# justinkay/aldi

Measured on AMD Instinct MI355X. Metric: images/sec (student+teacher ALDI step), R50-FPN 1333x800, higher is better.
Workload: dtype bf16

## Files before the change

### aldi_amd/csrc/elementwise.hip

```cpp
#include "common.h"
#include <stdlib.h>

namespace {

template <typename T>
__global__ void dgrad_weights_kernel(const float* __restrict__ w, const float* __restrict__ scale, T* __restrict__ wt,
                                     int Cout, int KH, int KW, int Cin) {
    long total = (long)Cout * KH * KW * Cin;
    for (long i = blockIdx.x * (long)blockDim.x + threadIdx.x; i < total; i += (long)gridDim.x * blockDim.x) {
        int co = (int)(i % Cout);
        long r = i / Cout;
        int kw = (int)(r % KW); r /= KW;
        int kh = (int)(r % KH);
        int ci = (int)(r / KH);
        float v = w[(((long)co * KH + (KH - 1 - kh)) * KW + (KW - 1 - kw)) * Cin + ci];
        if (scale) v *= scale[co];
        Elem<T>::st(wt + i, v);
    }
}

template <typename T>
__global__ __launch_bounds__(256) void dgrad_weights_batch_kernel(const aldi_dgw_item* __restrict__ items, int n_items) {
    __shared__ float tl[32][33];
    const int tile = blockIdx.x;
    int it = 0, hi = n_items - 1;
    while (it < hi) {
        const int mid = (it + hi + 1) >> 1;
        if (items[mid].tile_begin <= tile) it = mid;
        else hi = mid - 1;
    }
    const aldi_dgw_item d = items[it];
    const int Cout = d.Cout, KH = d.KH, KW = d.KW, Cin = d.Cin, T_ = KH * KW;
    const int nci = (Cin + 31) >> 5, nco = (Cout + 31) >> 5;
    int t = tile - d.tile_begin;
    const int cit = t % nci; t /= nci;
    const int cot = t % nco;
    const int tap = t / nco;
    const int kh = tap / KW, kw = tap - kh * KW;
    const int stap = (KH - 1 - kh) * KW + (KW - 1 - kw);
    const int tx = threadIdx.x & 31, ty = threadIdx.x >> 5;
#pragma unroll
    for (int k = 0; k < 4; ++k) {
        const int co = cot * 32 + ty + k * 8, ci = cit * 32 + tx;
        float v = 0.f;
        if (co < Cout && ci < Cin) {
            v = d.w_master[((long)co * T_ + stap) * Cin + ci];
            if (d.scale) v *= d.scale[co];
        }
        tl[ty + k * 8][tx] = v;
    }
    __syncthreads();
    T* __restrict__ wt = static_cast<T*>(d.wt);
#pragma unroll
    for (int k = 0; k < 4; ++k) {
        const int ci = cit * 32 + ty + k * 8, co = cot * 32 + tx;
        if (co < Cout && ci < Cin) Elem<T>::st(wt + ((long)ci * T_ + tap) * Cout + co, tl[tx][ty + k * 8]);
    }
}

struct StemDev {
    const uint8_t* img;
    const float* w;
    const float* scale; const float* shift;
    void* y;
    int N, Hs, Ws, Hc, Wc;
    int h[ALDI_MAX_IMAGES], wd[ALDI_MAX_IMAGES];
    float mean[3], inv_std[3];
};

template <typename T>
__global__ __launch_bounds__(256) void stem_kernel(StemDev p) {
    constexpr int TI = 16 * 2 + 5;
    __shared__ float ws[147 * 64];
    __shared__ float tile[3 * TI * TI];
    const int n = blockIdx.z;
    const int oy0 = blockIdx.y * 16, ox0 = blockIdx.x * 16;
    for (int i = threadIdx.x; i < 147 * 64; i += 256) {
        int co = i & 63, tap = i >> 6;
        ws[i] = p.w[co * 147 + tap];
    }
    const int iy0 = oy0 * 2 - 3, ix0 = ox0 * 2 - 3;
    const int h = p.h[n], w = p.wd[n];
    for (int i = threadIdx.x; i < 3 * TI * TI; i += 256) {
        int c = i / (TI * TI), r = i - c * TI * TI;
        int yy = r / TI, xx = r - yy * TI;
        int iy = iy0 + yy, ix = ix0 + xx;
        float v = 0.f;
        if (iy >= 0 && iy < h && ix >= 0 && ix < w)
            v = ((float)p.img[(((long)n * 3 + c) * p.Hs + iy) * p.Ws + ix] - p.mean[c]) * p.inv_std[c];
        tile[i] = v;
    }
    __syncthreads();
    const int ty = threadIdx.x >> 4, tx = threadIdx.x & 15;
    const int oy = oy0 + ty, ox = ox0 + tx;
    float acc[64];
#pragma unroll
    for (int i = 0; i < 64; ++i) acc[i] = 0.f;
    for (int kh = 0; kh < 7; ++kh)
        for (int kw = 0; kw < 7; ++kw)
#pragma unroll
            for (int c = 0; c < 3; ++c) {
                float xv = tile[(c * TI + ty * 2 + kh) * TI + tx * 2 + kw];
                const float4* wr = reinterpret_cast<const float4*>(&ws[((kh * 7 + kw) * 3 + c) * 64]);
#pragma unroll
                for (int q = 0; q < 16; ++q) {
                    float4 wv = wr[q];
                    acc[q * 4 + 0] = fmaf(xv, wv.x, acc[q * 4 + 0]);
                    acc[q * 4 + 1] = fmaf(xv, wv.y, acc[q * 4 + 1]);
                    acc[q * 4 + 2] = fmaf(xv, wv.z, acc[q * 4 + 2]);
                    acc[q * 4 + 3] = fmaf(xv, wv.w, acc[q * 4 + 3]);
                }
            }
    if (oy < p.Hc && ox < p.Wc) {
        T* out = static_cast<T*>(p.y) + (((long)n * p.Hc + oy) * p.Wc + ox) * 64;
#pragma unroll
        for (int q = 0; q < 16; ++q) {
            float v[4];
#pragma unroll
            for (int r = 0; r < 4; ++r) {
                float t = acc[q * 4 + r] * p.scale[q * 4 + r] + p.shift[q * 4 + r];
                v[r] = t > 0.f ? t : 0.f;
            }
            store4(out + q * 4, v);
        }
    }
}

__global__ __launch_bounds__(256) void stem_mfma_kernel(StemDev p) {
    constexpr int TH = 37, TW = 40, WK = 200;
    __shared__ __attribute__((aligned(16))) bf16_t wl[64 * WK];
    __shared__ __attribute__((aligned(16))) bf16_t tile[3 * TH * TW];
    const int n = blockIdx.z;
    const int oy0 = blockIdx.y * 16, ox0 = blockIdx.x * 16;
    for (int i = threadIdx.x; i < 64 * 192; i += 256) {
        const int co = i / 192, k = i - co * 192;
        const int idx = k >> 3, kw = k & 7;
        float v = 0.f;
        if (idx < 21 && kw < 7) {
            const int c = idx / 7, kh = idx - c * 7;
// ... 631 lines not shown
    }
    ALDI_CHECK_LAUNCH();
    return ALDI_OK;
}

extern "C" int aldi_upsample2_bwd(const void* g, void* out, int N, int Hc, int Wc, int C, int accumulate, int dtype, aldi_stream_t stream) {
    long total = (long)N * Hc * Wc * (C / 4);
    hipStream_t st = static_cast<hipStream_t>(stream);
    if (dtype == ALDI_BF16) hipLaunchKernelGGL(upsample2_bwd_kernel<bf16_t>, dim3(nblocks(total)), dim3(256), 0, st, (const bf16_t*)g, (bf16_t*)out, N, Hc, Wc, C, accumulate);
    else hipLaunchKernelGGL(upsample2_bwd_kernel<float>, dim3(nblocks(total)), dim3(256), 0, st, (const float*)g, (float*)out, N, Hc, Wc, C, accumulate);
    ALDI_CHECK_LAUNCH();
    return ALDI_OK;
}

extern "C" int aldi_upsample2_bwd_chain(const void* g2, void* o3, void* o4, void* o5, int N, int H5, int W5, int C, int dtype, aldi_stream_t stream) {
    if (!g2 || !o3 || !o4 || !o5 || N < 1 || H5 < 1 || W5 < 1 || (C & 3)) return aldi_set_error_msg(ALDI_ERR_ARG, "upsample2_bwd_chain: bad args");
    const long total = (long)N * H5 * W5 * (C / 4);
    hipStream_t st = static_cast<hipStream_t>(stream);
    if (dtype == ALDI_BF16) hipLaunchKernelGGL(upsample2_bwd_chain_kernel<bf16_t>, dim3(cdiv(total, 256)), dim3(256), 0, st, (const bf16_t*)g2, (bf16_t*)o3, (bf16_t*)o4, (bf16_t*)o5, N, H5, W5, C);
    else hipLaunchKernelGGL(upsample2_bwd_chain_kernel<float>, dim3(cdiv(total, 256)), dim3(256), 0, st, (const float*)g2, (float*)o3, (float*)o4, (float*)o5, N, H5, W5, C);
    ALDI_CHECK_LAUNCH();
    return ALDI_OK;
}

extern "C" int aldi_add_f32(const void* a, const float* b, const void* relu_src, void* out, long n, int dtype, aldi_stream_t stream) {
    if (n % 4) return aldi_set_error_msg(ALDI_ERR_ARG, "add_f32: n must be a multiple of 4");
    hipStream_t st = static_cast<hipStream_t>(stream);
    if (dtype == ALDI_BF16) hipLaunchKernelGGL(add_f32_kernel<bf16_t>, dim3(nblocks(n / 4)), dim3(256), 0, st, (const bf16_t*)a, b, (const bf16_t*)relu_src, (bf16_t*)out, n / 4);
    else hipLaunchKernelGGL(add_f32_kernel<float>, dim3(nblocks(n / 4)), dim3(256), 0, st, (const float*)a, b, (const float*)relu_src, (float*)out, n / 4);
    ALDI_CHECK_LAUNCH();
    return ALDI_OK;
}

extern "C" int aldi_cast_from_f32(const float* src, void* dst, long n, int dtype, aldi_stream_t stream) {
    hipStream_t st = static_cast<hipStream_t>(stream);
    if (dtype == ALDI_BF16) hipLaunchKernelGGL(cast_from_f32_kernel<bf16_t>, dim3(nblocks(n)), dim3(256), 0, st, src, (bf16_t*)dst, n);
    else hipLaunchKernelGGL(cast_from_f32_kernel<float>, dim3(nblocks(n)), dim3(256), 0, st, src, (float*)dst, n);
    ALDI_CHECK_LAUNCH();
    return ALDI_OK;
}

extern "C" int aldi_sgd_step(float* p, const float* g, float* buf, void* p_compute, long n, float lr, float momentum, float weight_decay,
                             float grad_scale, int first_step, int dtype, aldi_stream_t stream) {
    if (!p || !g || !buf) return aldi_set_error_msg(ALDI_ERR_ARG, "sgd_step: null pointer");
    hipStream_t st = static_cast<hipStream_t>(stream);
    if (dtype == ALDI_BF16) hipLaunchKernelGGL(sgd_kernel<bf16_t>, dim3(nblocks(n)), dim3(256), 0, st, p, g, buf, (bf16_t*)p_compute, n, lr, momentum, weight_decay, grad_scale, first_step);
    else hipLaunchKernelGGL(sgd_kernel<float>, dim3(nblocks(n)), dim3(256), 0, st, p, g, buf, (float*)nullptr, n, lr, momentum, weight_decay, grad_scale, first_step);
    ALDI_CHECK_LAUNCH();
    return ALDI_OK;
}

extern "C" int aldi_sgd_step_dev(float* p, const float* g, float* buf, void* p_compute, long n, const float* hyper, int dtype, aldi_stream_t stream) {
    if (!p || !g || !buf || !hyper || n <= 0) return aldi_set_error_msg(ALDI_ERR_ARG, "sgd_step_dev: bad args");
    hipStream_t st = static_cast<hipStream_t>(stream);
    if (dtype == ALDI_BF16) hipLaunchKernelGGL(sgd_dev_kernel<bf16_t>, dim3(nblocks(n)), dim3(256), 0, st, p, g, buf, (bf16_t*)p_compute, n, hyper);
    else hipLaunchKernelGGL(sgd_dev_kernel<float>, dim3(nblocks(n)), dim3(256), 0, st, p, g, buf, (float*)nullptr, n, hyper);
    ALDI_CHECK_LAUNCH();
    return ALDI_OK;
}

extern "C" int aldi_ema_update(float* teacher, const float* student, void* teacher_compute, long n, long n_compute, double alpha, int copy_only, int dtype,
                               aldi_stream_t stream) {
    if (!teacher || !student) return aldi_set_error_msg(ALDI_ERR_ARG, "ema_update: null pointer");
    hipStream_t st = static_cast<hipStream_t>(stream);
    const float oma = (float)(1.0 - alpha);
    const float alpha_f = (float)alpha;
    const long nc = teacher_compute ? (n_compute < n ? n_compute : n) : 0;
    const int cap = aldi_tuning().ema_blocks > 0 ? aldi_tuning().ema_blocks : 16384;
    if (dtype == ALDI_BF16) hipLaunchKernelGGL(ema_kernel<bf16_t>, dim3(nblocks(n / 4 + 1, 256, cap)), dim3(256), 0, st, teacher, student, (bf16_t*)teacher_compute, n, nc, oma, alpha_f, copy_only);
    else hipLaunchKernelGGL(ema_kernel<float>, dim3(nblocks(n / 4 + 1, 256, cap)), dim3(256), 0, st, teacher, student, (float*)nullptr, n, 0L, oma, alpha_f, copy_only);
    ALDI_CHECK_LAUNCH();
    return ALDI_OK;
}

extern "C" int aldi_bn_fold(const float* w, const float* b, const float* mean, const float* var, float* scale, float* shift, int C, aldi_stream_t stream) {
    hipLaunchKernelGGL(bn_fold_kernel, dim3(cdiv(C, 256)), dim3(256), 0, static_cast<hipStream_t>(stream), w, b, mean, var, scale, shift, C, 1e-5f);
    ALDI_CHECK_LAUNCH();
    return ALDI_OK;
}

extern "C" int aldi_dgrad_weights_batch(const aldi_dgw_item* items, int n_items, int total_tiles, int dtype, aldi_stream_t stream) {
    if (!items || n_items <= 0 || total_tiles <= 0) return aldi_set_error_msg(ALDI_ERR_ARG, "dgrad_weights_batch: bad args");
    hipStream_t st = static_cast<hipStream_t>(stream);
    if (dtype == ALDI_BF16) hipLaunchKernelGGL(dgrad_weights_batch_kernel<bf16_t>, dim3(total_tiles), dim3(256), 0, st, items, n_items);
    else if (dtype == ALDI_F32) hipLaunchKernelGGL(dgrad_weights_batch_kernel<float>, dim3(total_tiles), dim3(256), 0, st, items, n_items);
    else return aldi_set_error_msg(ALDI_ERR_ARG, "dgrad_weights_batch: bad dtype");
    ALDI_CHECK_LAUNCH();
    return ALDI_OK;
}

extern "C" int aldi_dgrad_weights(const float* w_master, const float* scale, void* wt, int Cout, int KH, int KW, int Cin,
                                  int dtype, aldi_stream_t stream) {
    if (!w_master || !wt) return aldi_set_error_msg(ALDI_ERR_ARG, "dgrad_weights: null pointer");
    long total = (long)Cout * KH * KW * Cin;
    int blocks = (int)((total + 255) / 256);
    if (blocks > 8192) blocks = 8192;
    hipStream_t st = static_cast<hipStream_t>(stream);
    if (dtype == ALDI_BF16) hipLaunchKernelGGL(dgrad_weights_kernel<bf16_t>, dim3(blocks), dim3(256), 0, st, w_master, scale, (bf16_t*)wt, Cout, KH, KW, Cin);
    else hipLaunchKernelGGL(dgrad_weights_kernel<float>, dim3(blocks), dim3(256), 0, st, w_master, scale, (float*)wt, Cout, KH, KW, Cin);
    ALDI_CHECK_LAUNCH();
    return ALDI_OK;
}
```

### aldi_amd/csrc/host.h

```cpp
#pragma once
#include "../../include/aldi_hip.h"

int aldi_set_error_msg(int code, const char* msg);

typedef uint16_t bf16_t;

#define ALDI_KNOBS(X) \
    X(igemm_xcd, 1) X(igemm_tile, 0) X(igemm_dbg, 0) X(igemm_bigtile_min, 1024) X(igemm_bigtile, 64) X(igemm_bigtile_k, 768) X(igemm_lintile_min, 768) \
    X(igemm_halo, 1) X(igemm_force, 0) X(igemm_k64_min, 1024) X(igemm_group, 1) X(igemm_narrow_k, 512) X(igemm_splitk_tile, 2) X(igemm_halo_f32, 0) \
    X(igemm_f32_tile64_max, 4096) X(igemm_direct, 15) X(igemm_lean, 1) X(igemm_halo64_mid, 0) X(igemm_ws, 1) X(igemm_ws_wgs, 512) X(igemm_ws_min, 40000) \
    X(wgrad_lean, 1) X(wgrad_big_min, 28) X(wgrad_big_slots, 256) X(wgrad_slots, 384) X(wgrad_xcd, 1) \
    X(igemm_halo_ilv, 1) X(igemm_halo_small, 0) X(igemm_halo96, 0) \
    X(wgrad_dma, 0) X(wgrad_dbg, 0) X(wgrad_group_slots, 0) X(wgrad_group_epi, 24) X(wgrad_db, 0) X(wgrad_ordered, 1) X(wgrad_big_group, 1) X(wgrad_big_epi, 12) \
    X(wgrad_big_group_min, 64) X(wgrad_lds_pad_kb, 0) X(wgrad_f32_tile128, 1) X(wgrad_dma64, 3) X(wgrad_ilv, 0) \
    X(msda_gather, 7) X(msda_gather_list, 1500) X(msda_bin, 1) X(msda_bin_list, 512) X(roialign_sep, 1) X(roialign_bwd_rows, 2) \
    X(colsum_blocks, 256) X(colsum_minrows, 16) X(colsum_nt, 1024) X(colsum_block_kb, 384) \
    X(stem_mfma, 1) X(stem_pool_wgs, 0) X(sab_blocks, 512) X(ln_bwd_blocks, 512) X(ln_bwd_blocks_narrow, 1024) X(rpn_topk_fused, 1) X(ema_blocks, 2048) X(nms_mask_tri, 1) X(match_wave, 1)

struct AldiTuning {
#define ALDI_KNOB_FIELD(name, dflt) int name;
    ALDI_KNOBS(ALDI_KNOB_FIELD)
#undef ALDI_KNOB_FIELD
};
AldiTuning& aldi_tuning();
void aldi_note_dispatch(const char* kernel);

static inline int cdiv(long a, long b) { return (int)((a + b - 1) / b); }
```

### aldi_amd/csrc/wgrad.hip

```cpp
#include "common.h"
#include "wgrad_select.h"
#include <hip/amd_detail/amd_hip_unsafe_atomics.h>
#include <stdio.h>
#include <stdlib.h>

namespace {

__device__ __forceinline__ int swz8(int row, int c) { return c ^ ((row >> 1) & 7); }

__device__ __forceinline__ void transpose8x8_b16(const uint4 in[8], uint4 out[8]) {
    const uint32_t* r = reinterpret_cast<const uint32_t*>(in);
    uint32_t* o = reinterpret_cast<uint32_t*>(out);
#pragma unroll
    for (int d = 0; d < 4; ++d)
#pragma unroll
        for (int j = 0; j < 4; ++j) {
            uint32_t a = r[(2 * j) * 4 + d], b = r[(2 * j + 1) * 4 + d];
            o[(2 * d) * 4 + j] = (a & 0xffffu) | (b << 16);
            o[(2 * d + 1) * 4 + j] = (a >> 16) | (b & 0xffff0000u);
        }
}

__global__ __launch_bounds__(256) void wgrad_bf16_kernel(WgDev p) {
    constexpr int BP = 64;
// ... 311 lines not shown
#pragma unroll
                for (int j = 0; j < 4; ++j) {
                    const uint32_t a = rr[(2 * j) * 4 + d], b = rr[(2 * j + 1) * 4 + d];
                    oo[(2 * d) * 4 + j] = __builtin_amdgcn_perm(b, a, 0x05040100u);
                    oo[(2 * d + 1) * 4 + j] = __builtin_amdgcn_perm(b, a, 0x07060302u);
                }
        }
        if constexpr (!DB) __syncthreads();
        uint4* img = DB ? lds + ((p0 - pbeg) / BP & 1) * ((TCO + TKK) * 8) : lds;
#pragma unroll
        for (int c = 0; c < 8; ++c) img[iw + c * 8 + (wu ^ (c >> 1))] = out[c];
        if (p0 + BP < pend) load_slab();
        __syncthreads();
#pragma unroll
        for (int ks = 0; ks < 2; ++ks) {
            uint4 af[TM], bfr[TN];
            const int ia = ia0 ^ (ks * 4), ib = ib0 ^ (ks * 4);
#pragma unroll
            for (int i = 0; i < TM; ++i) af[i] = img[ia + i * 128];
#pragma unroll
            for (int j = 0; j < TN; ++j) bfr[j] = img[ib + j * 128];
#pragma unroll
            for (int i = 0; i < TM; ++i)
#pragma unroll
                for (int j = 0; j < TN; ++j)
                    acc[i][j] = __builtin_amdgcn_mfma_f32_16x16x32_bf16(*reinterpret_cast<bf16x8_t*>(&af[i]),
                                                                         *reinterpret_cast<bf16x8_t*>(&bfr[j]), acc[i][j], 0, 0, 0);
            if (do_bias) {
#pragma unroll
                for (int i = 0; i < TM; ++i)
                    accb[i] = __builtin_amdgcn_mfma_f32_16x16x32_bf16(*reinterpret_cast<bf16x8_t*>(&af[i]), *reinterpret_cast<const bf16x8_t*>(&ones4), accb[i], 0, 0, 0);
            }
        }
    }
    wgrad_finish_tile<TCO, TKK, WM, WN>(p, acc, accb, do_bias, bx, by, bz, wave, lane);
}

__global__ __launch_bounds__(256) __attribute__((amdgpu_waves_per_eu(3))) void wgrad_bf16_lean_kernel(WgDev p) {
    __shared__ uint4 lds[2 * 128 * 8];
    wgrad_bf16_lean_body<128, 128, 2, 2>(p, lds);
}
__device__ __forceinline__ void wgrad_group_pick(const WgGroup& G, int& i, int& tx, int& ty, int& bz) {
    const int W = G.wg_begin[G.n];
    int g = (int)blockIdx.x;
    if (G.p[0].xcd) {
        const int q = W >> 3, r = W & 7, xcd = g & 7, idx = g >> 3;
        g = (xcd < r ? xcd * (q + 1) : r * (q + 1) + (xcd - r) * q) + idx;
    }
    i = 0;
    for (int k = 1; k < G.n; ++k)
        if (g >= G.wg_begin[k]) i = k;
    i = __builtin_amdgcn_readfirstlane(i);
    const int local = g - G.wg_begin[i];
    const int tiles = G.gx[i] * G.gy[i];
    const int t = local % tiles;
    bz = local / tiles;
    tx = t % G.gx[i]; ty = t / G.gx[i];
}
__global__ __launch_bounds__(256) __attribute__((amdgpu_waves_per_eu(3))) void wgrad_bf16_lean_group_kernel(WgGroup G) {
    __shared__ uint4 lds[2 * 128 * 8];
    int i, tx, ty, bz;
    wgrad_group_pick(G, i, tx, ty, bz);
    wgrad_bf16_lean_tile<128, 128, 2, 2>(G.p[i], lds, tx, ty, bz);
}

__global__ __launch_bounds__(256) void wgrad_bf16_lean_group_db_kernel(WgGroup G) {
    __shared__ uint4 lds[2 * 2 * 128 * 8];
    int i, tx, ty, bz;
    wgrad_group_pick(G, i, tx, ty, bz);
    wgrad_bf16_lean_tile<128, 128, 2, 2, true>(G.p[i], lds, tx, ty, bz);
}

__global__ __launch_bounds__(512) void wgrad_bf16_big_kernel(WgDev p) {
    __shared__ uint4 lds[2 * 256 * 8];
    wgrad_bf16_lean_body<256, 256, 2, 4>(p, lds);
}
__global__ __launch_bounds__(512) void wgrad_bf16_big_group_kernel(WgGroup G) {
    __shared__ uint4 lds[2 * 256 * 8];
    int i, tx, ty, bz;
    wgrad_group_pick(G, i, tx, ty, bz);
    wgrad_bf16_lean_tile<256, 256, 2, 4>(G.p[i], lds, tx, ty, bz);
}

template <int TCO, int TKK, int WM, int WN>
__device__ __forceinline__ void wgrad_finalize_part(const WgFinItem& it, int local) {
    constexpr int TM = TCO / WM / 16, TN = TKK / WN / 16, NW = WM * WN, NF = TM * TN, HALVES = NW / 4;
    const int S = it.S;
    const int nblk = it.gx * it.gy * NF * HALVES;
    if (local >= nblk) {
        if (!it.db || local > nblk) return;
        for (int co = threadIdx.x; co < it.Cout; co += 256) {
            const float* b = it.wsb + (long)(co / TCO) * S * TCO + co % TCO;
            float sum = 0.f;
            for (int k = 0; k < S; ++k) sum += b[(long)k * TCO];
            it.db[co] += sum;
        }
        return;
    }
    const int h = local % HALVES, f = (local / HALVES) % NF, t = local / (HALVES * NF);
    const int wave = h * 4 + (int)(threadIdx.x >> 6), lane = threadIdx.x & 63;
    const float4* src = reinterpret_cast<const float4*>(it.ws) + (((long)t * S) * NW + wave) * (long)(NF * 64) + f * 64 + lane;
    float4 sum = make_float4(0.f, 0.f, 0.f, 0.f);
    int k = 0;
    for (; k + 4 <= S; k += 4) {
        const float4 v0 = src[(long)(k + 0) * NW * NF * 64], v1 = src[(long)(k + 1) * NW * NF * 64];
        const float4 v2 = src[(long)(k + 2) * NW * NF * 64], v3 = src[(long)(k + 3) * NW * NF * 64];
        sum.x += v0.x; sum.y += v0.y; sum.z += v0.z; sum.w += v0.w;
        sum.x += v1.x; sum.y += v1.y; sum.z += v1.z; sum.w += v1.w;
        sum.x += v2.x; sum.y += v2.y; sum.z += v2.z; sum.w += v2.w;
        sum.x += v3.x; sum.y += v3.y; sum.z += v3.z; sum.w += v3.w;
    }
    for (; k < S; ++k) {
        const float4 v = src[(long)k * NW * NF * 64];
        sum.x += v.x; sum.y += v.y; sum.z += v.z; sum.w += v.w;
    }
    const int bx = t % it.gx, by = t / it.gx, wm = wave / WN, wn = wave % WN, i = f / TN, j = f % TN, fr = lane & 15, fq = lane >> 4;
    const int kk = by * TKK + wn * (TKK / WN) + j * 16 + fr;
    if (kk >= it.K) return;
    const float v[4] = {sum.x, sum.y, sum.z, sum.w};
#pragma unroll
    for (int r = 0; r < 4; ++r) {
        const int co = bx * TCO + wm * (TCO / WM) + i * 16 + fq * 4 + r;
        if (co < it.Cout) it.dw[(long)co * it.K + kk] += v[r] * (it.scale ? it.scale[co] : 1.f);
    }
}
__global__ __launch_bounds__(256) void wgrad_finalize_kernel(WgFin F) {
    const int bid = (int)blockIdx.x;
    int i = 0;
    for (int k = 1; k < F.n; ++k)
        if (bid >= F.wg_begin[k]) i = k;
    i = __builtin_amdgcn_readfirstlane(i);
    const int local = bid - F.wg_begin[i];
    if (F.it[i].big) wgrad_finalize_part<256, 256, 2, 4>(F.it[i], local);
    else wgrad_finalize_part<128, 128, 2, 2>(F.it[i], local);
}

typedef unsigned int u32x4 __attribute__((ext_vector_type(4)));
__device__ __forceinline__ void glds16w(__amdgpu_buffer_rsrc_t rsrc, void* dst, unsigned voff) {
    __builtin_amdgcn_raw_ptr_buffer_load_lds(rsrc, (__attribute__((address_space(3))) void*)dst, 16, voff, 0, 0, 0);
}
typedef unsigned int u32x2_t __attribute__((ext_vector_type(2)));
template <int OFF>
__device__ __forceinline__ u32x2_t tr_read(unsigned addr) {
    u32x2_t v;
    asm volatile("ds_read_b64_tr_b16 %0, %1 offset:%2" : "=v"(v) : "v"(addr), "n"(OFF));
    return v;
}
template <int N, int I = 0>
__device__ __forceinline__ void tr_read_frags(u32x2_t* lo, u32x2_t* hi, unsigned addr) {
    if constexpr (I < N) {
        lo[I] = tr_read<I * 1024>(addr);
        hi[I] = tr_read<I * 1024 + 512>(addr);
        tr_read_frags<N, I + 1>(lo, hi, addr);
    }
}

template <int TCO, int TKK, int WM, int WN>
__global__ __launch_bounds__(WM* WN * 64) void wgrad_bf16_dma_kernel(WgDev p) {
    constexpr int NW = WM * WN, NT = NW * 64;
    constexpr int BP = 32;
    constexpr int GB = TCO / 16, XB = TKK / 16;
    constexpr int NBLK = GB + XB;
    static_assert(NBLK % NW == 0, "every wave issues the same number of DMA instructions per slab");
    constexpr int PER_WAVE = NBLK / NW;
    constexpr int TM = TCO / WM / 16, TN = TKK / WN / 16;
    constexpr int NBUF = 3;
    constexpr int STAGE = NBLK * 1024;
    __shared__ __attribute__((aligned(1024))) unsigned char lds[NBUF * STAGE];

    const int tid = threadIdx.x, lane = tid & 63, wave = __builtin_amdgcn_readfirstlane(tid >> 6);
    int bx = blockIdx.x, by = blockIdx.y, bz = blockIdx.z;
    {
        const int gx = gridDim.x, gy = gridDim.y, total = gx * gy * gridDim.z;
        int bid = bx + gx * (by + gy * bz);
        if (p.xcd) {
            const int q = total >> 3, r = total & 7, xcd = bid & 7, idx = bid >> 3;
            bid = (xcd < r ? xcd * (q + 1) : r * (q + 1) + (xcd - r) * q) + idx;
        }
        bx = bid % gx; bid /= gx;
        by = bid % gy; bz = bid / gy;
    }
    const int co0 = bx * TCO, kk0 = by * TKK;
    const int pbeg = bz * p.pix_per_split;
    const int pend = min(p.M, pbeg + p.pix_per_split);
    if (pbeg >= pend) return;

    constexpr unsigned OOB = 0x80000000u;
    const __amdgpu_buffer_rsrc_t rg = make_rsrc_uniform(p.g, min((unsigned)pend * (unsigned)p.Cout * 2u, p.g_bytes));
    const __amdgpu_buffer_rsrc_t rx = make_rsrc_uniform(p.x, p.x_bytes);

    const int lp = lane >> 1, lh = lane & 1;
    unsigned voff[PER_WAVE];
    int tapbit[PER_WAVE];
#pragma unroll
    for (int k = 0; k < PER_WAVE; ++k) {
        const int b = wave * PER_WAVE + k;
        tapbit[k] = -1;
        if (b < GB) {
            const int ch = co0 + b * 16 + lh * 8;
            voff[k] = ch < p.Cout ? ((unsigned)(pbeg + lp) * (unsigned)p.Cout + (unsigned)ch) * 2u : OOB;
        } else {
            const int ch = kk0 + (b - GB) * 16 + lh * 8;
            if (ch >= p.K) { voff[k] = OOB; continue; }
            const int tap = ch / p.Cin, ci = ch - tap * p.Cin;
            const int kh = tap / p.KW, kw = tap - kh * p.KW;
            voff[k] = ((unsigned)(pbeg + lp + (kh - p.pad) * p.W + (kw - p.pad)) * (unsigned)p.Cin + (unsigned)ci) * 2u;
            if (!p.ident) tapbit[k] = tap;
        }
    }
    int ph = 0, pw = 0;
    if (!p.ident) {
        const int r = (pbeg + lp) % (p.H * p.W);
        ph = r / p.W; pw = r - ph * p.W;
    }
    const unsigned x_row = (unsigned)p.Cin * 2u, g_row = (unsigned)p.Cout * 2u;
    int ld_pix = pbeg;

// ... 508 lines not shown
    float acc[EP];
#pragma unroll
    for (int k = 0; k < EP; ++k) acc[k] = 0.f;
    auto add = [&](const uint4& v) {
        if constexpr (EP == 8) {
            const uint32_t* w = reinterpret_cast<const uint32_t*>(&v);
#pragma unroll
            for (int k = 0; k < 4; ++k) { acc[2 * k] += __uint_as_float(w[k] << 16); acc[2 * k + 1] += __uint_as_float(w[k] & 0xffff0000u); }
        } else {
            const float* w = reinterpret_cast<const float*>(&v);
#pragma unroll
            for (int k = 0; k < 4; ++k) acc[k] += w[k];
        }
    };
    if (lane_r < rl) {
        const T* __restrict__ col = g + ch * EP;
        int r = r0 + lane_r;
        for (; r + 3 * rl < r1; r += 4 * rl) {
            const uint4 v0 = *reinterpret_cast<const uint4*>(col + (long)r * ld);
            const uint4 v1 = *reinterpret_cast<const uint4*>(col + (long)(r + rl) * ld);
            const uint4 v2 = *reinterpret_cast<const uint4*>(col + (long)(r + 2 * rl) * ld);
            const uint4 v3 = *reinterpret_cast<const uint4*>(col + (long)(r + 3 * rl) * ld);
            add(v0); add(v1); add(v2); add(v3);
        }
        for (; r < r1; r += rl) add(*reinterpret_cast<const uint4*>(col + (long)r * ld));
    }
#pragma unroll
    for (int k = 0; k < EP; ++k) red[threadIdx.x * EP + k] = acc[k];
    __syncthreads();
    for (int c = threadIdx.x; c < C; c += NT) {
        const int cch = c / EP, k = c % EP;
        float s = 0.f;
        for (int l = 0; l < rl; ++l) s += red[(l * chunks + cch) * EP + k];
        if (s != 0.f) unsafeAtomicAdd(db + c, s);
    }
}

WgPlan& plan_storage() {
    static thread_local WgPlan P;
    return P;
}

int execute_plan(const WgPlan& P, hipStream_t st) {
    for (const WgLaunch& L : P.launches) {
        const dim3 grid(L.gx, L.gy, L.gz), block(kWgForms[L.form].threads);
        const WgDev& d = L.d;
        const WgGroup& G = P.groups[L.group];
        switch (L.form) {
        case WG_GENERIC: hipLaunchKernelGGL(wgrad_bf16_kernel, grid, block, 0, st, d); break;
        case WG_LEAN: hipLaunchKernelGGL(wgrad_bf16_lean_kernel, grid, block, 0, st, d); break;
        case WG_BIG: hipLaunchKernelGGL(wgrad_bf16_big_kernel, grid, block, 0, st, d); break;
        case WG_BIG64:
            if (L.ilv) hipLaunchKernelGGL(wgrad_bf16_big64_kernel<true>, grid, block, 0, st, d);
            else hipLaunchKernelGGL(wgrad_bf16_big64_kernel<false>, grid, block, 0, st, d);
            break;
        case WG_DMA: hipLaunchKernelGGL((wgrad_bf16_dma_kernel<128, 128, 2, 2>), grid, block, 0, st, d); break;
        case WG_F32: hipLaunchKernelGGL(wgrad_f32_kernel, grid, block, 0, st, d); break;
        case WG_F32_T128: hipLaunchKernelGGL(wgrad_f32_t128_kernel<32>, grid, block, 0, st, d); break;
        case WG_LEAN_GROUP: hipLaunchKernelGGL(wgrad_bf16_lean_group_kernel, grid, block, (size_t)L.lds, st, G); break;
        case WG_LEAN_GROUP_DB: hipLaunchKernelGGL(wgrad_bf16_lean_group_db_kernel, grid, block, 0, st, G); break;
        case WG_LEAN64_GROUP:
            if (L.ilv) hipLaunchKernelGGL(wgrad_bf16_lean64_group_kernel<true>, grid, block, 0, st, G);
            else hipLaunchKernelGGL(wgrad_bf16_lean64_group_kernel<false>, grid, block, 0, st, G);
            break;
        case WG_BIG_GROUP: hipLaunchKernelGGL(wgrad_bf16_big_group_kernel, grid, block, 0, st, G); break;
        case WG_BIG64_GROUP:
            if (L.ilv) hipLaunchKernelGGL(wgrad_bf16_big64_group_kernel<true>, grid, block, 0, st, G);
            else hipLaunchKernelGGL(wgrad_bf16_big64_group_kernel<false>, grid, block, 0, st, G);
            break;
        default: return aldi_set_error_msg(ALDI_ERR_ARG, "conv_wgrad: bad launch form");
        }
        ALDI_CHECK_LAUNCH();
        if (L.bias_pass)
            if (int rc = aldi_bias_grad(d.g, d.db, d.M, d.Cout, L.dtype, st)) return rc;
    }
    for (size_t i0 = 0; i0 < P.fin.size(); i0 += kMaxGroup) {
        WgFin F;
        F.n = (int)(P.fin.size() - i0 < (size_t)kMaxGroup ? P.fin.size() - i0 : kMaxGroup);
        int wg = 0;
        for (int k = 0; k <= kMaxGroup; ++k) {
            F.wg_begin[k] = wg;
            if (k < F.n) { F.it[k] = P.fin[i0 + k]; wg += fin_workgroups(F.it[k]); }
        }
        hipLaunchKernelGGL(wgrad_finalize_kernel, dim3(wg), dim3(256), 0, st, F);
        ALDI_CHECK_LAUNCH();
    }
    char name[200];
    dispatch_name(P, name, sizeof(name));
    aldi_note_dispatch(name);
    return ALDI_OK;
}

}

extern "C" int aldi_conv_wgrad_group(const aldi_wgrad_args* args, int n, aldi_stream_t stream) {
    WgPlan& P = plan_storage();
    if (int rc = plan_wgrad(args, n, true, false, aldi_tuning(), P)) return rc;
    return execute_plan(P, static_cast<hipStream_t>(stream));
}
extern "C" long aldi_conv_wgrad_group_workspace(const aldi_wgrad_args* args, int n) { return workspace_bytes(args, n, aldi_tuning(), plan_storage()); }

extern "C" int aldi_conv_wgrad(const aldi_wgrad_args* a, aldi_stream_t stream) {
    WgPlan& P = plan_storage();
    if (int rc = plan_wgrad(a, 1, false, false, aldi_tuning(), P)) return rc;
    return execute_plan(P, static_cast<hipStream_t>(stream));
}

extern "C" int aldi_conv_wgrad_plan(const aldi_wgrad_args* args, int n, int group, char* name, int cap, long* ws_bytes) {
    WgPlan& P = plan_storage();
    if (int rc = plan_wgrad(args, n, group != 0, false, aldi_tuning(), P)) return rc;
    char buf[200];
    dispatch_name(P, buf, sizeof(buf));
    if (ws_bytes && (*ws_bytes = workspace_bytes(args, group ? n : 1, aldi_tuning(), P)) < 0) return ALDI_ERR_ARG;
    if (name && cap > 0) snprintf(name, (size_t)cap, "%s", buf);
    return ALDI_OK;
}

extern "C" int aldi_bias_grad(const void* g, float* db, int M, int C, int dtype, aldi_stream_t stream) {
    if (!g || !db || M <= 0 || C <= 0) return aldi_set_error_msg(ALDI_ERR_ARG, "bias_grad: bad args");
    hipStream_t st = static_cast<hipStream_t>(stream);
    const int ep = dtype == ALDI_BF16 ? 8 : 4;
    if (C % ep) return aldi_set_error_msg(ALDI_ERR_ARG, "bias_grad: C must be a multiple of a 16-B chunk");
    const AldiTuning& tn = aldi_tuning();
    const int target_blocks = tn.colsum_blocks, min_rows = tn.colsum_minrows, nt_env = tn.colsum_nt, block_kb = tn.colsum_block_kb;
    const long row_bytes = (long)C * (dtype == ALDI_BF16 ? 2 : 4);
    int rows_per_block = cdiv(M, target_blocks);
    const int by_bytes = (int)(((long)block_kb << 10) / row_bytes);
    if (rows_per_block < by_bytes) rows_per_block = by_bytes;
    if (rows_per_block < min_rows) rows_per_block = min_rows;
    dim3 grid(cdiv(M, rows_per_block));
    for (int c0 = 0; c0 < C; c0 += 256 * ep) {
        const int cs = C - c0 < 256 * ep ? C - c0 : 256 * ep;
        if (dtype == ALDI_BF16) {
            if (nt_env == 1024) hipLaunchKernelGGL((colsum_kernel<bf16_t, 1024>), grid, dim3(1024), 0, st, (const bf16_t*)g + c0, db + c0, M, cs, C, rows_per_block);
            else hipLaunchKernelGGL((colsum_kernel<bf16_t, 256>), grid, dim3(256), 0, st, (const bf16_t*)g + c0, db + c0, M, cs, C, rows_per_block);
        } else hipLaunchKernelGGL((colsum_kernel<float, 256>), grid, dim3(256), 0, st, (const float*)g + c0, db + c0, M, cs, C, rows_per_block);
    }
    ALDI_CHECK_LAUNCH();
    return ALDI_OK;
}
```

Baseline: 511.8.

## Batch dgrad weight transpose into persistent chunks and ring-prefetch wgrad finalize

The dgrad weight flip/transpose kernel now runs a capped grid in which each block walks a contiguous chunk of tiles, processes 64x32 tiles where possible, and writes packed bf16 pairs as 32-bit stores. The wgrad split-K finalize gains a ring-buffered reduction with 8 loads in flight, and it hoists the dw/scale reads ahead of the reduction so their latency overlaps. Both target memory latency and launch overhead in small bandwidth-bound kernels. The cost is more complex tile indexing, extra syncthreads per unit, and higher register use.

```diff
diff --git a/aldi_amd/csrc/elementwise.hip b/aldi_amd/csrc/elementwise.hip
--- a/aldi_amd/csrc/elementwise.hip
+++ b/aldi_amd/csrc/elementwise.hip
@@ -20,41 +20,81 @@
 }
 
 template <typename T>
-__global__ __launch_bounds__(256) void dgrad_weights_batch_kernel(const aldi_dgw_item* __restrict__ items, int n_items) {
-    __shared__ float tl[32][33];
-    const int tile = blockIdx.x;
+__device__ __forceinline__ void dgw_unit(const aldi_dgw_item& d, float (*tl)[33], int tap, int co0, int ci0, int rows, bool packed) {
+    const int Cout = d.Cout, Cin = d.Cin, T_ = d.KH * d.KW;
+    const int kh = tap / d.KW, kw = tap - kh * d.KW;
+    const int stap = (d.KH - 1 - kh) * d.KW + (d.KW - 1 - kw);
+    const int tx = threadIdx.x & 31, ty = threadIdx.x >> 5;
+    const int ci = ci0 + tx;
+    float v[8], sc[8];
+#pragma unroll
+    for (int k = 0; k < 8; ++k) {
+        const int r = ty + k * 8, co = co0 + r;
+        v[k] = 0.f; sc[k] = 1.f;
+        if (r < rows && co < Cout && ci < Cin) {
+            v[k] = d.w_master[((long)co * T_ + stap) * Cin + ci];
+            if (d.scale) sc[k] = d.scale[co];
+        }
+    }
+#pragma unroll
+    for (int k = 0; k < 8; ++k)
+        if (ty + k * 8 < rows) tl[ty + k * 8][tx] = d.scale ? v[k] * sc[k] : v[k];
+    __syncthreads();
+    T* __restrict__ wt = static_cast<T*>(d.wt);
+    if constexpr (sizeof(T) == 2) {
+        if (packed) {
+            const int cl = 2 * tx, co = co0 + cl;
+#pragma unroll
+            for (int k = 0; k < 4; ++k) {
+                const int cr = ty + k * 8, cc = ci0 + cr;
+                if (cl < rows && co < Cout && cc < Cin)
+                    *reinterpret_cast<uint32_t*>(wt + ((long)cc * T_ + tap) * Cout + co) = pack2_bf16(tl[cl][cr], tl[cl + 1][cr]);
+            }
+            __syncthreads();
+            return;
+        }
+    }
+    const int cl = threadIdx.x & 63, co = co0 + cl, cy = threadIdx.x >> 6;
+#pragma unroll
+    for (int k = 0; k < 8; ++k) {
+        const int cr = cy + k * 4, cc = ci0 + cr;
+        if (cl < rows && co < Cout && cc < Cin) Elem<T>::st(wt + ((long)cc * T_ + tap) * Cout + co, tl[cl][cr]);
+    }
+    __syncthreads();
+}
+
+template <typename T>
+__global__ __launch_bounds__(256) void dgrad_weights_batch_kernel(const aldi_dgw_item* __restrict__ items, int n_items, int total_tiles, int chunk) {
+    __shared__ float tl[64][33];
+    const long lo_ = (long)blockIdx.x * chunk;
+    if (lo_ >= total_tiles) return;
+    const int lo = (int)lo_, hi_t = (int)(lo_ + chunk < total_tiles ? lo_ + chunk : total_tiles);
     int it = 0, hi = n_items - 1;
     while (it < hi) {
         const int mid = (it + hi + 1) >> 1;
-        if (items[mid].tile_begin <= tile) it = mid;
+        if (items[mid].tile_begin <= lo) it = mid;
         else hi = mid - 1;
     }
-    const aldi_dgw_item d = items[it];
-    const int Cout = d.Cout, KH = d.KH, KW = d.KW, Cin = d.Cin, T_ = KH * KW;
-    const int nci = (Cin + 31) >> 5, nco = (Cout + 31) >> 5;
-    int t = tile - d.tile_begin;
-    const int cit = t % nci; t /= nci;
-    const int cot = t % nco;
-    const int tap = t / nco;
-    const int kh = tap / KW, kw = tap - kh * KW;
-    const int stap = (KH - 1 - kh) * KW + (KW - 1 - kw);
-    const int tx = threadIdx.x & 31, ty = threadIdx.x >> 5;
-#pragma unroll
-    for (int k = 0; k < 4; ++k) {
-        const int co = cot * 32 + ty + k * 8, ci = cit * 32 + tx;
-        float v = 0.f;
-        if (co < Cout && ci < Cin) {
-            v = d.w_master[((long)co * T_ + stap) * Cin + ci];
-            if (d.scale) v *= d.scale[co];
-        }
-        tl[ty + k * 8][tx] = v;
-    }
-    __syncthreads();
-    T* __restrict__ wt = static_cast<T*>(d.wt);
-#pragma unroll
-    for (int k = 0; k < 4; ++k) {
-        const int ci = cit * 32 + ty + k * 8, co = cot * 32 + tx;
-        if (co < Cout && ci < Cin) Elem<T>::st(wt + ((long)ci * T_ + tap) * Cout + co, tl[tx][ty + k * 8]);
+    int t = lo;
+    while (t < hi_t) {
+        while (it + 1 < n_items && items[it + 1].tile_begin <= t) ++it;
+        const aldi_dgw_item d = items[it];
+        const int next = it + 1 < n_items ? items[it + 1].tile_begin : total_tiles;
+        const int nci = (d.Cin + 31) >> 5, nco = (d.Cout + 31) >> 5, per_tap = nco * nci;
+        int l = t - d.tile_begin;
+        int lend = (next < hi_t ? next : hi_t) - d.tile_begin;
+        t = d.tile_begin + lend;
+        if (lend > d.KH * d.KW * per_tap) lend = d.KH * d.KW * per_tap;
+        const bool packed = sizeof(T) == 2 && (d.Cout & 1) == 0 && ((uintptr_t)d.wt & 3) == 0;
+        while (l < lend) {
+            const int tap = l / per_tap, s = l - tap * per_tap;
+            const int p = s / (2 * nci), r = s - p * 2 * nci;
+            const bool full = 2 * p + 1 < nco;
+            const int cit = full ? r >> 1 : r, half = full ? r & 1 : 0;
+            const bool two = full && half == 0 && l + 1 < lend;
+            dgw_unit<T>(d, tl, tap, (2 * p + half) * 32, cit * 32, two ? 64 : 32, packed);
+            l += two ? 2 : 1;
+        }
     }
 }
 
@@ -852,8 +892,10 @@
 extern "C" int aldi_dgrad_weights_batch(const aldi_dgw_item* items, int n_items, int total_tiles, int dtype, aldi_stream_t stream) {
     if (!items || n_items <= 0 || total_tiles <= 0) return aldi_set_error_msg(ALDI_ERR_ARG, "dgrad_weights_batch: bad args");
     hipStream_t st = static_cast<hipStream_t>(stream);
-    if (dtype == ALDI_BF16) hipLaunchKernelGGL(dgrad_weights_batch_kernel<bf16_t>, dim3(total_tiles), dim3(256), 0, st, items, n_items);
-    else if (dtype == ALDI_F32) hipLaunchKernelGGL(dgrad_weights_batch_kernel<float>, dim3(total_tiles), dim3(256), 0, st, items, n_items);
+    const int chunk = 2 * cdiv(total_tiles, 2 * 2048);
+    const dim3 grid(cdiv(total_tiles, chunk));
+    if (dtype == ALDI_BF16) hipLaunchKernelGGL(dgrad_weights_batch_kernel<bf16_t>, grid, dim3(256), 0, st, items, n_items, total_tiles, chunk);
+    else if (dtype == ALDI_F32) hipLaunchKernelGGL(dgrad_weights_batch_kernel<float>, grid, dim3(256), 0, st, items, n_items, total_tiles, chunk);
     else return aldi_set_error_msg(ALDI_ERR_ARG, "dgrad_weights_batch: bad dtype");
     ALDI_CHECK_LAUNCH();
     return ALDI_OK;
diff --git a/aldi_amd/csrc/host.h b/aldi_amd/csrc/host.h
--- a/aldi_amd/csrc/host.h
+++ b/aldi_amd/csrc/host.h
@@ -12,7 +12,7 @@
     X(wgrad_lean, 1) X(wgrad_big_min, 28) X(wgrad_big_slots, 256) X(wgrad_slots, 384) X(wgrad_xcd, 1) \
     X(igemm_halo_ilv, 1) X(igemm_halo_small, 0) X(igemm_halo96, 0) \
     X(wgrad_dma, 0) X(wgrad_dbg, 0) X(wgrad_group_slots, 0) X(wgrad_group_epi, 24) X(wgrad_db, 0) X(wgrad_ordered, 1) X(wgrad_big_group, 1) X(wgrad_big_epi, 12) \
-    X(wgrad_big_group_min, 64) X(wgrad_lds_pad_kb, 0) X(wgrad_f32_tile128, 1) X(wgrad_dma64, 3) X(wgrad_ilv, 0) \
+    X(wgrad_big_group_min, 64) X(wgrad_lds_pad_kb, 0) X(wgrad_f32_tile128, 1) X(wgrad_dma64, 3) X(wgrad_ilv, 0) X(wgrad_fin_ring, 1) \
     X(msda_gather, 7) X(msda_gather_list, 1500) X(msda_bin, 1) X(msda_bin_list, 512) X(roialign_sep, 1) X(roialign_bwd_rows, 2) \
     X(colsum_blocks, 256) X(colsum_minrows, 16) X(colsum_nt, 1024) X(colsum_block_kb, 384) \
     X(stem_mfma, 1) X(stem_pool_wgs, 0) X(sab_blocks, 512) X(ln_bwd_blocks, 512) X(ln_bwd_blocks_narrow, 1024) X(rpn_topk_fused, 1) X(ema_blocks, 2048) X(nms_mask_tri, 1) X(match_wave, 1)
diff --git a/aldi_amd/csrc/wgrad.hip b/aldi_amd/csrc/wgrad.hip
--- a/aldi_amd/csrc/wgrad.hip
+++ b/aldi_amd/csrc/wgrad.hip
@@ -417,57 +417,116 @@
     wgrad_bf16_lean_tile<256, 256, 2, 4>(G.p[i], lds, tx, ty, bz);
 }
 
-template <int TCO, int TKK, int WM, int WN>
+__device__ __forceinline__ void fin_add(float4& s, const float4& v) { s.x += v.x; s.y += v.y; s.z += v.z; s.w += v.w; }
+__device__ __forceinline__ void fin_add(float& s, float v) { s += v; }
+template <int R, typename V>
+__device__ __forceinline__ V fin_ordered_sum(const V* __restrict__ src, long stride, int S) {
+    V sum, ring[R], tail[R - 1];
+    __builtin_memset(&sum, 0, sizeof(V));
+    const bool full = S >= R;
+    int k = 0;
+    if (full) {
+#pragma unroll
+        for (int j = 0; j < R; ++j) ring[j] = src[(long)j * stride];
+        for (; k + 2 * R <= S; k += R) {
+#pragma unroll
+            for (int j = 0; j < R; ++j) {
+                fin_add(sum, ring[j]);
+                ring[j] = src[(long)(k + R + j) * stride];
+            }
+        }
+        k += R;
+    }
+    const int rem = S - k;
+#pragma unroll
+    for (int j = 0; j < R - 1; ++j) {
+        __builtin_memset(&tail[j], 0, sizeof(V));
+        if (j < rem) tail[j] = src[(long)(k + j) * stride];
+    }
+    if (full) {
+#pragma unroll
+        for (int j = 0; j < R; ++j) fin_add(sum, ring[j]);
+    }
+#pragma unroll
+    for (int j = 0; j < R - 1; ++j)
+        if (j < rem) fin_add(sum, tail[j]);
+    return sum;
+}
+
+template <int TCO, int TKK, int WM, int WN, bool RING>
 __device__ __forceinline__ void wgrad_finalize_part(const WgFinItem& it, int local) {
     constexpr int TM = TCO / WM / 16, TN = TKK / WN / 16, NW = WM * WN, NF = TM * TN, HALVES = NW / 4;
+    constexpr int R = 8;
     const int S = it.S;
     const int nblk = it.gx * it.gy * NF * HALVES;
     if (local >= nblk) {
         if (!it.db || local > nblk) return;
         for (int co = threadIdx.x; co < it.Cout; co += 256) {
             const float* b = it.wsb + (long)(co / TCO) * S * TCO + co % TCO;
-            float sum = 0.f;
-            for (int k = 0; k < S; ++k) sum += b[(long)k * TCO];
-            it.db[co] += sum;
+            if constexpr (RING) {
+                const float old = it.db[co];
+                it.db[co] = old + fin_ordered_sum<R, float>(b, TCO, S);
+            } else {
+                float sum = 0.f;
+                for (int k = 0; k < S; ++k) sum += b[(long)k * TCO];
+                it.db[co] += sum;
+            }
         }
         return;
     }
     const int h = local % HALVES, f = (local / HALVES) % NF, t = local / (HALVES * NF);
     const int wave = h * 4 + (int)(threadIdx.x >> 6), lane = threadIdx.x & 63;
     const float4* src = reinterpret_cast<const float4*>(it.ws) + (((long)t * S) * NW + wave) * (long)(NF * 64) + f * 64 + lane;
-    float4 sum = make_float4(0.f, 0.f, 0.f, 0.f);
-    int k = 0;
-    for (; k + 4 <= S; k += 4) {
-        const float4 v0 = src[(long)(k + 0) * NW * NF * 64], v1 = src[(long)(k + 1) * NW * NF * 64];
-        const float4 v2 = src[(long)(k + 2) * NW * NF * 64], v3 = src[(long)(k + 3) * NW * NF * 64];
-        sum.x += v0.x; sum.y += v0.y; sum.z += v0.z; sum.w += v0.w;
-        sum.x += v1.x; sum.y += v1.y; sum.z += v1.z; sum.w += v1.w;
-        sum.x += v2.x; sum.y += v2.y; sum.z += v2.z; sum.w += v2.w;
-        sum.x += v3.x; sum.y += v3.y; sum.z += v3.z; sum.w += v3.w;
-    }
-    for (; k < S; ++k) {
-        const float4 v = src[(long)k * NW * NF * 64];
-        sum.x += v.x; sum.y += v.y; sum.z += v.z; sum.w += v.w;
-    }
     const int bx = t % it.gx, by = t / it.gx, wm = wave / WN, wn = wave % WN, i = f / TN, j = f % TN, fr = lane & 15, fq = lane >> 4;
     const int kk = by * TKK + wn * (TKK / WN) + j * 16 + fr;
-    if (kk >= it.K) return;
-    const float v[4] = {sum.x, sum.y, sum.z, sum.w};
-#pragma unroll
-    for (int r = 0; r < 4; ++r) {
-        const int co = bx * TCO + wm * (TCO / WM) + i * 16 + fq * 4 + r;
-        if (co < it.Cout) it.dw[(long)co * it.K + kk] += v[r] * (it.scale ? it.scale[co] : 1.f);
-    }
-}
+    const int co0 = bx * TCO + wm * (TCO / WM) + i * 16 + fq * 4;
+    if constexpr (RING) {
+        float old[4], sc[4];
+#pragma unroll
+        for (int r = 0; r < 4; ++r) {
+            const bool ok = kk < it.K && co0 + r < it.Cout;
+            old[r] = ok ? it.dw[(long)(co0 + r) * it.K + kk] : 0.f;
+            sc[r] = ok && it.scale ? it.scale[co0 + r] : 1.f;
+        }
+        const float4 sum = fin_ordered_sum<R, float4>(src, (long)NW * NF * 64, S);
+        if (kk >= it.K) return;
+        const float v[4] = {sum.x, sum.y, sum.z, sum.w};
+#pragma unroll
+        for (int r = 0; r < 4; ++r)
+            if (co0 + r < it.Cout) it.dw[(long)(co0 + r) * it.K + kk] = old[r] + v[r] * sc[r];
+    } else {
+        float4 sum = make_float4(0.f, 0.f, 0.f, 0.f);
+        int k = 0;
+        for (; k + 4 <= S; k += 4) {
+            const float4 v0 = src[(long)(k + 0) * NW * NF * 64], v1 = src[(long)(k + 1) * NW * NF * 64];
+            const float4 v2 = src[(long)(k + 2) * NW * NF * 64], v3 = src[(long)(k + 3) * NW * NF * 64];
+            sum.x += v0.x; sum.y += v0.y; sum.z += v0.z; sum.w += v0.w;
+            sum.x += v1.x; sum.y += v1.y; sum.z += v1.z; sum.w += v1.w;
+            sum.x += v2.x; sum.y += v2.y; sum.z += v2.z; sum.w += v2.w;
+            sum.x += v3.x; sum.y += v3.y; sum.z += v3.z; sum.w += v3.w;
+        }
+        for (; k < S; ++k) {
+            const float4 v = src[(long)k * NW * NF * 64];
+            sum.x += v.x; sum.y += v.y; sum.z += v.z; sum.w += v.w;
+        }
+        if (kk >= it.K) return;
+        const float v[4] = {sum.x, sum.y, sum.z, sum.w};
+#pragma unroll
+        for (int r = 0; r < 4; ++r) {
+            const int co = co0 + r;
+            if (co < it.Cout) it.dw[(long)co * it.K + kk] += v[r] * (it.scale ? it.scale[co] : 1.f);
+        }
+    }
+}
+template <bool RING>
 __global__ __launch_bounds__(256) void wgrad_finalize_kernel(WgFin F) {
     const int bid = (int)blockIdx.x;
     int i = 0;
-    for (int k = 1; k < F.n; ++k)
-        if (bid >= F.wg_begin[k]) i = k;
+    for (int k = 1; k < F.n && bid >= F.wg_begin[k]; ++k) i = k;
     i = __builtin_amdgcn_readfirstlane(i);
     const int local = bid - F.wg_begin[i];
-    if (F.it[i].big) wgrad_finalize_part<256, 256, 2, 4>(F.it[i], local);
-    else wgrad_finalize_part<128, 128, 2, 2>(F.it[i], local);
+    if (F.it[i].big) wgrad_finalize_part<256, 256, 2, 4, RING>(F.it[i], local);
+    else wgrad_finalize_part<128, 128, 2, 2, RING>(F.it[i], local);
 }
 
 typedef unsigned int u32x4 __attribute__((ext_vector_type(4)));
@@ -1142,7 +1201,8 @@
             F.wg_begin[k] = wg;
             if (k < F.n) { F.it[k] = P.fin[i0 + k]; wg += fin_workgroups(F.it[k]); }
         }
-        hipLaunchKernelGGL(wgrad_finalize_kernel, dim3(wg), dim3(256), 0, st, F);
+        if (aldi_tuning().wgrad_fin_ring) hipLaunchKernelGGL(wgrad_finalize_kernel<true>, dim3(wg), dim3(256), 0, st, F);
+        else hipLaunchKernelGGL(wgrad_finalize_kernel<false>, dim3(wg), dim3(256), 0, st, F);
         ALDI_CHECK_LAUNCH();
     }
     char name[200];
```

Result: no change. 509.9 (-0.4%).
